# flavie-yuan-liu/DL_attack_on_ImageNet

Measured on AMD Instinct MI355X. Metric: adversarial images/sec (ADiL learning step, classifier included), higher is better.
Workload: dtype bf16; 1 GPU; ADiL learn_dictionary_a step vs resnet50, 512 images/GPU, 50 atoms, 224x224, bf16 image streams + fp32 D/V master, loss=logits, clean pseudo-labels computed once per image and cached (1 fwd + 1 bwd per step; result-neutral, profiles/r03_label_stability.md); global_batch=512, atoms=50, inner_iters=131, parallelism=dp1: images+codes sharded, D replicated, 1 all-reduce(grad_d)/step

## Files before the change

### dl_attack_on_imagenet_amd/_lib.py

```python
import ctypes
import os
from ctypes import c_float, c_int, c_size_t, c_void_p

_PKG = os.path.dirname(os.path.abspath(__file__))
LIBPATH = os.environ.get("ADIL_HIP_LIBRARY") or os.path.join(_PKG, "lib", "libadil_hip.so")

SIGNATURES = {
    "adil_abi_version": (c_int, []),
    "adil_max_atoms": (c_int, []),
    "adil_grad_workspace_bytes": (c_size_t, [c_int, c_int, c_int]),
    "adil_grad_code_rows": (c_int, [c_int]),
    "adil_grad_slab_offset": (c_size_t, [c_int, c_int, c_int]),
    "adil_pack_codes": (c_int, [c_void_p, c_void_p, c_int, c_int, c_void_p, c_void_p, c_void_p, c_int, c_void_p, c_int, c_int,
                                c_void_p]),
    "adil_gather_images": (c_int, [c_void_p, c_int, c_void_p, c_void_p, c_int, c_int, c_int, c_void_p]),
    "adil_spd_inverse": (c_int, [c_void_p, c_int, c_void_p, c_void_p]),
    "adil_synth": (c_int, [c_void_p, c_void_p, c_void_p, c_void_p, c_int, c_int, c_int, c_int, c_float, c_int, c_void_p]),
    "adil_images_to_u8": (c_int, [c_void_p, c_int, c_void_p, c_size_t, c_void_p, c_void_p]),
    "adil_synth_store": (c_int, [c_void_p, c_void_p, c_void_p, c_void_p, c_void_p, c_int, c_int, c_int, c_int, c_float, c_int,
                                 c_void_p]),
    "adil_synth_fp8": (c_int, [c_void_p, c_void_p, c_void_p, c_void_p, c_int, c_int, c_int, c_int, c_float, c_float, c_int,
                               c_void_p]),
    "adil_dict_to_fp8": (c_int, [c_void_p, c_size_t, c_void_p, c_void_p]),
    "adil_adamw_clamp_fp8": (c_int, [c_void_p, c_void_p, c_int, c_void_p, c_void_p, c_size_t, c_float, c_float, c_float,
                                     c_float, c_float, c_float, c_float, c_float, c_void_p, c_void_p, c_void_p, c_void_p]),
    "adil_synth_fp8_packed": (c_int, [c_void_p, c_void_p, c_void_p, c_void_p, c_int, c_int, c_int, c_int, c_float, c_float,
                                      c_int, c_void_p]),
    "adil_grad": (c_int, [c_void_p, c_void_p, c_void_p, c_void_p, c_void_p, c_void_p, c_int, c_int, c_int, c_int, c_int,
                          c_void_p, c_size_t, c_void_p, c_void_p]),
    "adil_adamw_clamp": (c_int, [c_void_p, c_void_p, c_int, c_void_p, c_void_p, c_size_t, c_float, c_float, c_float,
                                 c_float, c_float, c_float, c_float, c_float, c_void_p, c_void_p, c_void_p]),
    "adil_zstep": (c_int, [c_void_p, c_void_p, c_void_p, c_void_p, c_void_p, c_int, c_int, c_int, c_float, c_float,
                           c_float, c_float, c_float, c_float, c_float, c_float, c_void_p, c_void_p, c_float, c_void_p,
                           c_void_p, c_void_p]),
    "adil_zstep_codes_slab_bytes": (c_size_t, [c_int, c_int, c_int]),
    "adil_zstep_codes": (c_int, [c_void_p, c_void_p, c_void_p, c_void_p, c_void_p, c_int, c_int, c_int, c_float, c_float,
                                 c_float, c_float, c_float, c_float, c_float, c_float, c_void_p, c_void_p, c_float, c_void_p,
                                 c_void_p, c_void_p, c_size_t, c_void_p, c_void_p]),
    "adil_adamw_l1ball": (c_int, [c_void_p, c_void_p, c_void_p, c_int, c_void_p, c_void_p, c_int, c_int, c_float, c_float,
                                  c_float, c_float, c_float, c_float, c_float, c_void_p, c_void_p, c_float, c_void_p, c_void_p,
                                  c_void_p, c_int, c_int, c_void_p]),
    "adil_atom_l1ball_project": (c_int, [c_void_p, c_int, c_int, c_int, c_float, c_void_p]),
    "adil_l1ball_project": (c_int, [c_void_p, c_int, c_int, c_float, c_void_p]),
    "adil_l2ball_project": (c_int, [c_void_p, c_int, c_int, c_float, c_void_p]),
    "adil_ista_step": (c_int, [c_void_p, c_void_p, c_size_t, c_float, c_float, c_void_p]),
    "adil_atom_workspace_bytes": (c_size_t, [c_int, c_int]),
    "adil_atom_norms": (c_int, [c_void_p, c_int, c_int, c_void_p, c_void_p, c_size_t, c_void_p]),
    "adil_atom_scale": (c_int, [c_void_p, c_int, c_int, c_void_p, c_int, c_void_p]),
    "adil_gram_workspace_bytes": (c_size_t, [c_int, c_int]),
    "adil_gram": (c_int, [c_void_p, c_int, c_int, c_void_p, c_void_p, c_size_t, c_void_p]),
    "adil_dict_rightmul": (c_int, [c_void_p, c_void_p, c_int, c_int, c_void_p, c_void_p]),
    "adil_image_metrics": (c_int, [c_void_p, c_void_p, c_int, c_int, c_int, c_void_p, c_void_p, c_void_p]),
    "adil_affine_act_fwd": (c_int, [c_void_p, c_void_p, c_void_p, c_void_p, c_void_p, c_size_t, c_int, c_int, c_int, c_int,
                                    c_void_p]),
    "adil_affine_act_bwd": (c_int, [c_void_p, c_void_p, c_void_p, c_void_p, c_void_p, c_size_t, c_int, c_int, c_int, c_int,
                                    c_void_p]),
    "adil_stem_conv_fwd": (c_int, [c_void_p, c_int, c_void_p, c_float, c_float, c_float, c_float, c_float, c_float,
                                   c_void_p, c_void_p, c_void_p, c_int, c_int, c_int, c_void_p]),
    "adil_maxpool_fwd": (c_int, [c_void_p, c_void_p, c_void_p, c_int, c_int, c_int, c_int, c_void_p]),
    "adil_stem_pool_bwd": (c_int, [c_void_p, c_void_p, c_void_p, c_void_p, c_void_p, c_int, c_int, c_int, c_int, c_void_p]),
    "adil_pw_conv_fwd": (c_int, [c_void_p, c_void_p, c_void_p, c_void_p, c_void_p, c_void_p, c_int, c_int, c_int, c_int,
                                 c_void_p, c_void_p, c_int, c_int, c_void_p]),
    "adil_pw_conv_bwd": (c_int, [c_void_p, c_void_p, c_void_p, c_void_p, c_void_p, c_void_p, c_void_p, c_int, c_int, c_int,
                                 c_int, c_void_p, c_void_p, c_void_p, c_void_p, c_int, c_int, c_void_p]),
    "adil_pw_conv_bwd_tile": (c_int, [c_void_p, c_void_p, c_void_p, c_void_p, c_void_p, c_void_p, c_void_p, c_int, c_int, c_int,
                                      c_int, c_void_p, c_void_p, c_void_p, c_void_p, c_int, c_int, c_void_p, c_int]),
    "adil_pw_route_policy": (c_int, [c_int]),
    "adil_pw_join_fwd": (c_int, [c_void_p, c_void_p, c_void_p, c_void_p, c_void_p, c_void_p, c_void_p, c_void_p, c_void_p,
                                 c_void_p, c_void_p, c_void_p, c_int, c_int, c_int, c_void_p]),
    "adil_pw_join_bwd": (c_int, [c_void_p, c_void_p, c_void_p, c_void_p, c_void_p, c_void_p, c_void_p, c_void_p, c_void_p,
                                 c_void_p, c_void_p, c_void_p, c_void_p, c_int, c_int, c_int, c_void_p]),
    "adil_conv3x3": (c_int, [c_void_p, c_void_p, c_void_p, c_int, c_int, c_int, c_int, c_int, c_void_p]),
    "adil_conv3x3_loop": (c_int, [c_int]),
    "adil_conv3x3_s2_fwd": (c_int, [c_void_p, c_void_p, c_void_p, c_int, c_int, c_int, c_int, c_int, c_void_p]),
    "adil_conv3x3_s2_bwd": (c_int, [c_void_p, c_void_p, c_void_p, c_int, c_int, c_int, c_int, c_int, c_void_p]),
    "adil_dw3x3_fwd": (c_int, [c_void_p, c_void_p, c_void_p, c_void_p, c_int, c_int, c_int, c_int, c_int, c_int, c_void_p]),
    "adil_dw3x3_bwd": (c_int, [c_void_p, c_void_p, c_void_p, c_void_p, c_int, c_int, c_int, c_int, c_int, c_int, c_void_p]),
    "adil_pw8_fwd": (c_int, [c_void_p, c_void_p, c_void_p, c_void_p, c_void_p, c_void_p, c_int, c_int, c_int, c_int, c_void_p]),
    "adil_pw8_bwd": (c_int, [c_void_p, c_void_p, c_void_p, c_void_p, c_void_p, c_int, c_int, c_int, c_int, c_void_p]),
    "adil_stem_conv_bwd": (c_int, [c_void_p, c_void_p, c_float, c_float, c_float, c_void_p, c_int, c_int, c_int, c_int,
                                   c_void_p]),
    "adil_stem_bwd_variant": (c_int, [c_int]),
    "adil_first3x3_fwd": (c_int, [c_void_p, c_int, c_void_p, c_float, c_float, c_float, c_float, c_float, c_float,
                                  c_void_p, c_void_p, c_void_p, c_int, c_int, c_int, c_int, c_void_p]),
    "adil_first3x3_bwd": (c_int, [c_void_p, c_void_p, c_void_p, c_void_p, c_float, c_float, c_float, c_void_p, c_int, c_int,
                                  c_int, c_int, c_int, c_void_p]),
    "adil_pool_head_fwd": (c_int, [c_void_p, c_void_p, c_void_p, c_void_p, c_void_p, c_int, c_int, c_int, c_int, c_void_p]),
    "adil_pool_head_bwd": (c_int, [c_void_p, c_void_p, c_void_p, c_void_p, c_int, c_int, c_int, c_int, c_void_p]),
    "adil_bn_pool_head_fwd": (c_int, [c_void_p] * 7 + [c_int, c_int, c_int, c_int, c_void_p]),
    "adil_bn_pool_head_bwd": (c_int, [c_void_p] * 7 + [c_int, c_int, c_int, c_int, c_void_p]),
    "adil_dense1x1_fwd": (c_int, [c_void_p, c_void_p, c_void_p, c_void_p, c_void_p, c_void_p, c_void_p, c_int, c_int, c_int,
                                  c_int, c_void_p]),
    "adil_dense1x1_bwd": (c_int, [c_void_p, c_void_p, c_void_p, c_void_p, c_void_p, c_void_p, c_void_p, c_void_p, c_int, c_int,
                                  c_int, c_int, c_void_p]),
    "adil_dense3x3_fwd": (c_int, [c_void_p, c_void_p, c_void_p, c_int, c_int, c_int, c_int, c_int, c_void_p]),
    "adil_dense3x3_bwd": (c_int, [c_void_p, c_void_p, c_void_p, c_int, c_int, c_int, c_int, c_int, c_void_p]),
    "adil_dense1x1_fwd_ld": (c_int, [c_void_p, c_int, c_void_p, c_void_p, c_void_p, c_void_p, c_void_p, c_void_p, c_int, c_int,
                                     c_int, c_int, c_int, c_void_p]),
    "adil_dense1x1_bwd_ld": (c_int, [c_void_p, c_int, c_void_p, c_int, c_void_p, c_void_p, c_void_p, c_int, c_void_p, c_void_p,
                                     c_void_p, c_int, c_int, c_int, c_int, c_int, c_int, c_void_p]),
    "adil_dense3x3_fwd_ld": (c_int, [c_void_p, c_int, c_void_p, c_void_p, c_int, c_int, c_int, c_int, c_int, c_int, c_void_p]),
    "adil_dense3x3_bwd_ld": (c_int, [c_void_p, c_int, c_void_p, c_void_p, c_int, c_int, c_int, c_int, c_int, c_int, c_void_p]),
    "adil_dense_transition_fwd": (c_int, [c_void_p, c_void_p, c_void_p, c_void_p, c_void_p, c_int, c_int, c_int, c_int, c_int,
                                          c_void_p]),
    "adil_dense_transition_bwd": (c_int, [c_void_p, c_int, c_void_p, c_void_p, c_void_p, c_void_p, c_void_p, c_int, c_int,
                                          c_int, c_int, c_int, c_void_p]),
}

ABI_VERSION = 8
_lib = None


class AdilLibraryError(RuntimeError):
    pass


def load(path: str = None) -> ctypes.CDLL:
    global _lib
    if _lib is not None and path is None:
        return _lib
    p = path or LIBPATH
    import torch
    if not os.path.exists(p):
        raise AdilLibraryError(
            f"HIP kernel library not found at {p}. Build it with `python -m dl_attack_on_imagenet_amd.build` "
            "(needs hipcc). There is no CPU fallback for the ADiL hot path.")
# ... 22 lines not shown
```

### dl_attack_on_imagenet_amd/csrc/adil_convs.hip

```cpp
#include <hip/hip_runtime.h>
#include <stdint.h>

#include "adil_common.h"
#include "adil_hip.h"
#include "adil_mfma.h"

namespace {

#define PW_BM 128
#define PW_BK 64
#define PW_LS (PW_BK + 8)
#define PW_PK 512

template <int BN, bool PRO, bool RES>
__global__ __launch_bounds__(256) __attribute__((amdgpu_waves_per_eu(PRO && BN == 128 ? 2 : (RES ? 3 : 4)))) void pw_conv_fwd_kernel(
    const bf16_t* __restrict__ x, const bf16_t* __restrict__ wgt, const float* __restrict__ scale,
    const float* __restrict__ shift, const bf16_t* __restrict__ res, bf16_t* __restrict__ y, int M, int K, int N,
    int relu, int MT, int NT, const float* __restrict__ pscale, const float* __restrict__ pshift, int sub_w, int sub_hw) {
    constexpr int CT = BN / 32;
    constexpr int XCH = PW_BM * PW_BK / 8 / 256;
    constexpr int WCH = BN * PW_BK / 8 / 256;
    constexpr int OS = BN + 8;
    extern __shared__ __attribute__((aligned(16))) unsigned char smem_raw[];
    bf16_t* sx = reinterpret_cast<bf16_t*>(smem_raw);
// ... 695 lines not shown
}

template <int WD, bool BWD>
int launch_pw_join(const JoinArgs& a, hipStream_t st) {
    const size_t lds = ((size_t)(PW_BM + 64) * (WD + 8) + (size_t)(WD + PW_BM) * PW_LS) * sizeof(bf16_t);
    if (lds > 48 * 1024) {
        const hipError_t e = hipFuncSetAttribute((const void*)pw_join_kernel<WD, BWD>,
                                                 hipFuncAttributeMaxDynamicSharedMemorySize, (int)lds);
        if (e != hipSuccess) return (int)e;
    }
    hipLaunchKernelGGL((pw_join_kernel<WD, BWD>), dim3((unsigned)((a.M + PW_BM - 1) / PW_BM)), dim3(256), lds, st, a);
    ADIL_CHECK_LAUNCH();
    return 0;
}

template <bool BWD>
int launch_pw_join_w(const JoinArgs& a, int W, hipStream_t st) {
    if (W == 64) return launch_pw_join<64, BWD>(a, st);
    return launch_pw_join<128, BWD>(a, st);
}

}

extern "C" int adil_pw_join_fwd(const void* h2raw, const float* pscale2, const float* pshift2, const void* w3,
                                const float* scale3, const float* shift3, const void* res, void* out, const void* w1,
                                const float* scale1, const float* shift1, void* h1, int M, int W, int C, void* stream) {
    ADIL_ENTER();
    if (!h2raw || !pscale2 || !pshift2 || !w3 || !scale3 || !shift3 || !res || !out || !w1 || !scale1 || !shift1 || !h1 ||
        M <= 0 || (W != 64 && W != 128) || C != 4 * W)
        return ADIL_EINVAL;
    const JoinArgs a = {(const bf16_t*)h2raw, nullptr, pscale2, pshift2, (const bf16_t*)w3, scale3, shift3,
                        (const bf16_t*)res, nullptr, (bf16_t*)out, (const bf16_t*)w1, scale1, shift1, nullptr, (bf16_t*)h1,
                        M, C};
    return launch_pw_join_w<false>(a, W, (hipStream_t)stream);
}

extern "C" int adil_pw_join_bwd(const void* g_h1, const void* h1, const float* scale1, const void* wt1, const void* g_out,
                                const void* out, const float* scale3, void* gres, const void* wt3, const void* h2raw,
                                const float* pscale2, const float* pshift2, void* gx, int M, int W, int C, void* stream) {
    ADIL_ENTER();
    if (!g_h1 || !h1 || !scale1 || !wt1 || !g_out || !out || !scale3 || !gres || !wt3 || !h2raw || !pscale2 || !pshift2 ||
        !gx || M <= 0 || (W != 64 && W != 128) || C != 4 * W)
        return ADIL_EINVAL;
    const JoinArgs a = {(const bf16_t*)g_h1, (const bf16_t*)h1, scale1, nullptr, (const bf16_t*)wt1, scale3, nullptr,
                        (const bf16_t*)g_out, (const bf16_t*)out, (bf16_t*)gres, (const bf16_t*)wt3, pscale2, pshift2,
                        (const bf16_t*)h2raw, (bf16_t*)gx, M, C};
    return launch_pw_join_w<true>(a, W, (hipStream_t)stream);
}

namespace {

#define C3_LS 72

template <int BN, int WPX, int LOOP>
__global__ __launch_bounds__(256) __attribute__((amdgpu_waves_per_eu(2))) void conv3x3_kernel(
    const bf16_t* __restrict__ x, const bf16_t* __restrict__ wp, bf16_t* __restrict__ y, int M, int H, int W, int C, int N,
    int MT, int NT) {
    constexpr int C3_BM = WPX * 64;
    constexpr int CTW = BN / 32 / (4 / WPX);
    constexpr int XCHK = (C3_BM + 128) * 8 / 256;
    constexpr int WCH = BN * 8 / 256;
    constexpr int OS = BN + 8;
    extern __shared__ __attribute__((aligned(16))) unsigned char smem_raw[];
    const int NP = C3_BM + 2 * W + 2;
    bf16_t* sx = reinterpret_cast<bf16_t*>(smem_raw);
    const int sx_elems = (NP * C3_LS > C3_BM * OS ? NP * C3_LS : C3_BM * OS);
    bf16_t* sw = sx + ((sx_elems + 7) & ~7);
    const int tid = threadIdx.x, lane = tid & 63, w = tid >> 6, c = lane & 31, h = lane >> 5;
    const int wpx = w % WPX, wch = w / WPX;
    int mt, nt;
    if ((MT & 7) == 0) {
        const int xcd = blockIdx.x & 7, j = blockIdx.x >> 3;
        nt = j % NT;
        mt = (j / NT) * 8 + xcd;
    } else {
        nt = blockIdx.x % NT;
        mt = blockIdx.x / NT;
    }
    const int m0 = mt * C3_BM, n0 = nt * BN;
    const int nci = C >> 6;

    int pl[2];
    unsigned vmask[2];
#pragma unroll
    for (int p = 0; p < 2; ++p) {
        pl[p] = (wpx * 2 + p) * 32 + c;
        const int m = m0 + pl[p];
        const int ww = m % W, hh = (m / W) % H;
        unsigned vm = 0;
#pragma unroll
        for (int t = 0; t < 9; ++t) {
            const int kh = t / 3, kw = t - 3 * kh;
            const bool ok = (m < M) && (hh + kh - 1 >= 0) && (hh + kh - 1 < H) && (ww + kw - 1 >= 0) && (ww + kw - 1 < W);
            vm |= ok ? (1u << t) : 0u;
        }
        vmask[p] = vm;
    }

    u32x4 xr[XCHK], wr[3][WCH];
    [[maybe_unused]] auto load_x = [&](int cc) {
#pragma unroll
        for (int i = 0; i < XCHK; ++i) {
            const int q = tid + 256 * i, px = q >> 3, ch = q & 7;
            int gm = m0 - W - 1 + (px < NP ? px : NP - 1);
            gm = gm < 0 ? 0 : (gm >= M ? M - 1 : gm);
            xr[i] = *reinterpret_cast<const u32x4*>(x + (size_t)gm * C + cc * 64 + ch * 8);
        }
    };
    auto store_x = [&]() {
#pragma unroll
        for (int i = 0; i < XCHK; ++i) {
            const int q = tid + 256 * i, px = q >> 3, ch = q & 7;
            if (px < NP) *reinterpret_cast<u32x4*>(sx + px * C3_LS + ch * 8) = xr[i];
        }
    };
    const int nit = nci * 9;
    [[maybe_unused]] auto load_w = [&](int it, u32x4 (&r)[WCH]) {
        const int itc = it < nit ? it : nit - 1;
        const int cc = itc / 9, tap = itc - 9 * cc;
#pragma unroll
        for (int i = 0; i < WCH; ++i) {
            const int q = tid + 256 * i, row = q >> 3, ch = q & 7;
            r[i] = *reinterpret_cast<const u32x4*>(wp + ((size_t)(n0 + row) * 9 + tap) * C + cc * 64 + ch * 8);
        }
    };
    auto store_w = [&](int buf, const u32x4 (&r)[WCH]) {
#pragma unroll
        for (int i = 0; i < WCH; ++i) {
            const int q = tid + 256 * i, row = q >> 3, ch = q & 7;
            *reinterpret_cast<u32x4*>(sw + (buf * BN + row) * C3_LS + ch * 8) = r[i];
        }
    };

    f32x16 acc[2][CTW];
#pragma unroll
    for (int p = 0; p < 2; ++p)
#pragma unroll
        for (int ct = 0; ct < CTW; ++ct)
#pragma unroll
            for (int r = 0; r < 16; ++r) acc[p][ct][r] = 0.0f;

    if constexpr (LOOP == 1) {
        auto tap_body = [&](int it, u32x4 (&rfree)[WCH], const u32x4 (&rnext)[WCH]) {
            const int buf = it & 1;
            const int cc = it / 9, tap = it - 9 * cc;
            const int kh = tap / 3, kw = tap - 3 * kh;
            load_w(it + 3, rfree);
            if (tap == 4 && cc + 1 < nci) load_x(cc + 1);
            const bf16_t* bw = sw + (buf * BN + (wch * CTW) * 32 + c) * C3_LS + 8 * h;
            const int shift = kh * W + kw;
            const bool ok0 = (vmask[0] >> tap) & 1u, ok1 = (vmask[1] >> tap) & 1u;
#pragma unroll
            for (int ks = 0; ks < 4; ++ks) {
                bf16x8 b0 = lds8(sx + (pl[0] + shift) * C3_LS + 16 * ks + 8 * h);
                bf16x8 b1 = lds8(sx + (pl[1] + shift) * C3_LS + 16 * ks + 8 * h);
                u32x4 z0 = __builtin_bit_cast(u32x4, b0), z1 = __builtin_bit_cast(u32x4, b1);
#pragma unroll
                for (int j = 0; j < 4; ++j) { z0[j] = ok0 ? z0[j] : 0u; z1[j] = ok1 ? z1[j] : 0u; }
                b0 = __builtin_bit_cast(bf16x8, z0);
                b1 = __builtin_bit_cast(bf16x8, z1);
#pragma unroll
                for (int ct = 0; ct < CTW; ++ct) {
                    const bf16x8 a = lds8(bw + ct * 32 * C3_LS + 16 * ks);
                    mma16(acc[0][ct], a, b0);
                    mma16(acc[1][ct], a, b1);
                }
            }
            if (it + 1 < nit) store_w(buf ^ 1, rnext);
            if (tap == 8 && cc + 1 < nci) {
                lds_barrier();
                store_x();
            }
            lds_barrier();
        };

        load_x(0);
        load_w(0, wr[0]);
        load_w(1, wr[1]);
        load_w(2, wr[2]);
        store_x();
        store_w(0, wr[0]);
        __syncthreads();
        for (int it = 0; it < nit; it += 3) {
            tap_body(it, wr[0], wr[1]);
            tap_body(it + 1, wr[1], wr[2]);
            tap_body(it + 2, wr[2], wr[0]);
        }
    } else {
        const unsigned wq = (((unsigned)(n0 + (tid >> 3)) * 9u) * (unsigned)C + (unsigned)(tid & 7) * 8u) * 2u;
        const size_t wrow = (size_t)32 * 9 * C;
        auto load_w0 = [&](unsigned ws, u32x4 (&r)[WCH]) {
#pragma unroll
            for (int i = 0; i < WCH; ++i)
                r[i] = *reinterpret_cast<const u32x4*>(reinterpret_cast<const char*>(wp + ws + i * wrow) + wq);
        };
        const int gmb = m0 - W - 1 > 0 ? m0 - W - 1 : 0;
        const bf16_t* xb = x + (size_t)gmb * C;
        unsigned xq[XCHK];
#pragma unroll
        for (int i = 0; i < XCHK; ++i) {
            const int px = (tid >> 3) + 32 * i;
            int gm = m0 - W - 1 + (px < NP ? px : NP - 1);
            gm = gm < 0 ? 0 : (gm >= M ? M - 1 : gm);
            xq[i] = ((unsigned)(gm - gmb) * (unsigned)C + (unsigned)(tid & 7) * 8u) * 2u;
        }
        auto load_x0 = [&](int cc) {
#pragma unroll
            for (int i = 0; i < XCHK; ++i)
                xr[i] = *reinterpret_cast<const u32x4*>(reinterpret_cast<const char*>(xb + cc * 64) + xq[i]);
        };
        bf16_t* sz = sw + 2 * BN * C3_LS;
        const bf16_t* xl0 = sx + pl[0] * C3_LS + 8 * h;
        const bf16_t* xl1 = sx + pl[1] * C3_LS + 8 * h;
        const bf16_t* zl = sz + 8 * h;
        const bf16_t* bwl = sw + ((wch * CTW) * 32 + c) * C3_LS + 8 * h;
        auto xrow = [&](const bf16_t* xl, unsigned vm, int tap) -> const bf16_t* {
            const int kh = tap / 3, kw = tap - 3 * kh;
            const bf16_t* a = xl + (kh * W + kw) * C3_LS;
            if (tap == 4) return a;
            return (vm & (1u << tap)) ? a : zl;
        };
        struct Frag {
            bf16x8 b0, b1, a[CTW];
        };
        auto read_frag = [&](Frag& f, const bf16_t* p0, const bf16_t* p1, const bf16_t* bw, int ks) {
            f.b0 = lds8(p0 + 16 * ks);
            f.b1 = lds8(p1 + 16 * ks);
#pragma unroll
            for (int ct = 0; ct < CTW; ++ct) f.a[ct] = lds8(bw + ct * 32 * C3_LS + 16 * ks);
        };
        auto mma_frag = [&](const Frag& f) {
#pragma unroll
            for (int ct = 0; ct < CTW; ++ct) {
                mma16(acc[0][ct], f.a[ct], f.b0);
                mma16(acc[1][ct], f.a[ct], f.b1);
            }
        };

        load_x0(0);
        load_w0(0u, wr[0]);
        load_w0((unsigned)C, wr[1]);
        load_w0(2u * (unsigned)C, wr[2]);
        store_x();
        store_w(0, wr[0]);
        if (tid < C3_LS / 8) reinterpret_cast<u32x4*>(sz)[tid] = u32x4{0u, 0u, 0u, 0u};
        __syncthreads();
        Frag fa, fb;
        const bf16_t* p0 = xrow(xl0, vmask[0], 0);
        const bf16_t* p1 = xrow(xl1, vmask[1], 0);
        read_frag(fa, p0, p1, bwl, 0);
        for (int cc = 0; cc < nci; ++cc) {
            const bool more = cc + 1 < nci;
            const unsigned wsc = (unsigned)cc * 64u, wsn = (unsigned)(more ? cc + 1 : cc) * 64u;
#pragma unroll
            for (int tap = 0; tap < 9; ++tap) {
                const int buf = (cc + tap) & 1;
                const bf16_t* bw = bwl + buf * BN * C3_LS;
                const bool last = !more && tap == 8;
                read_frag(fb, p0, p1, bw, 1);
                if (!last) store_w(buf ^ 1, wr[(tap + 1) % 3]);
                load_w0(tap + 3 < 9 ? wsc + (unsigned)((tap + 3) * C) : wsn + (unsigned)((tap - 6) * C), wr[tap % 3]);
                if (tap == 4 && more) load_x0(cc + 1);
                __builtin_amdgcn_sched_barrier(0);
                mma_frag(fa);
                __builtin_amdgcn_sched_barrier(0);
                read_frag(fa, p0, p1, bw, 2);
                __builtin_amdgcn_sched_barrier(0);
                mma_frag(fb);
                __builtin_amdgcn_sched_barrier(0);
                read_frag(fb, p0, p1, bw, 3);
                __builtin_amdgcn_sched_barrier(0);
                mma_frag(fa);
                __builtin_amdgcn_sched_barrier(0);
                lds_barrier();
                if (tap == 8 && more) {
                    store_x();
                    lds_barrier();
                }
                if (!last) {
                    p0 = xrow(xl0, vmask[0], (tap + 1) % 9);
                    p1 = xrow(xl1, vmask[1], (tap + 1) % 9);
                    read_frag(fa, p0, p1, bwl + (buf ^ 1) * BN * C3_LS, 0);
                }
                __builtin_amdgcn_sched_barrier(0);
                mma_frag(fb);
                __builtin_amdgcn_sched_barrier(0);
            }
        }
    }
#pragma unroll
    for (int p = 0; p < 2; ++p) {
#pragma unroll
        for (int ct = 0; ct < CTW; ++ct) {
#pragma unroll
            for (int q = 0; q < 4; ++q) {
                u32x2 t;
                t[0] = pack2_bf16(acc[p][ct][4 * q], acc[p][ct][4 * q + 1]);
                t[1] = pack2_bf16(acc[p][ct][4 * q + 2], acc[p][ct][4 * q + 3]);
                *reinterpret_cast<u32x2*>(sx + pl[p] * OS + (wch * CTW + ct) * 32 + 8 * q + 4 * h) = t;
            }
        }
    }
    __syncthreads();
    constexpr int CPP = BN / 8;
#pragma unroll
    for (int i = 0; i < C3_BM * CPP / 256; ++i) {
        const int id = tid + 256 * i, px = id / CPP, ch = id - px * CPP;
        const int mm = m0 + px;
        if (mm < M) *reinterpret_cast<u32x4*>(y + (size_t)mm * N + n0 + ch * 8) = *reinterpret_cast<const u32x4*>(sx + px * OS + ch * 8);
    }
}

template <int BN, int WPX, int LOOP>
int launch_conv3x3(const void* x, const void* wp, void* y, int M, int H, int W, int C, int N, hipStream_t st) {
    constexpr int C3_BM = WPX * 64;
    const int MT = (M + C3_BM - 1) / C3_BM, NT = N / BN;
    const int NP = C3_BM + 2 * W + 2;
    size_t sx_elems = (size_t)NP * C3_LS;
    if (sx_elems < (size_t)C3_BM * (BN + 8)) sx_elems = (size_t)C3_BM * (BN + 8);
    sx_elems = (sx_elems + 7) & ~(size_t)7;
    const size_t lds = (sx_elems + (size_t)2 * BN * C3_LS + (LOOP == 0 ? C3_LS : 0)) * sizeof(bf16_t);
    if (lds > 160 * 1024) return ADIL_EINVAL;
    if (lds > 48 * 1024) {
        const hipError_t e = hipFuncSetAttribute((const void*)conv3x3_kernel<BN, WPX, LOOP>,
                                                 hipFuncAttributeMaxDynamicSharedMemorySize, (int)lds);
        if (e != hipSuccess) return (int)e;
    }
    hipLaunchKernelGGL((conv3x3_kernel<BN, WPX, LOOP>), dim3((unsigned)(MT * NT)), dim3(256), lds, st, (const bf16_t*)x,
                       (const bf16_t*)wp, (bf16_t*)y, M, H, W, C, N, MT, NT);
    ADIL_CHECK_LAUNCH();
    return 0;
}

static int g_conv3x3_loop = 0;

}

extern "C" int adil_conv3x3_loop(int variant) {
    const int prev = g_conv3x3_loop;
    if (variant == 0 || variant == 1) g_conv3x3_loop = variant;
    return prev;
}

extern "C" int adil_conv3x3(const void* x, const void* wp, void* y, int B, int H, int W, int C, int N, void* stream) {
    ADIL_ENTER();
    if (!x || !wp || !y || B <= 0 || H <= 0 || W <= 0 || C <= 0 || N <= 0 || (C % 64) || (N % 64) || W > 63) return ADIL_EINVAL;
    const long long M = (long long)B * H * W;
    if (M > 0x7fffffffLL) return ADIL_EINVAL;
    if (9LL * C * N > 0x7fffffffLL) return ADIL_EINVAL;
    const hipStream_t st = (hipStream_t)stream;
    if (g_conv3x3_loop == 1) {
        if (N % 128 == 0) return launch_conv3x3<128, 2, 1>(x, wp, y, (int)M, H, W, C, N, st);
        return launch_conv3x3<64, 4, 1>(x, wp, y, (int)M, H, W, C, N, st);
    }
    if (N % 128 == 0) return launch_conv3x3<128, 2, 0>(x, wp, y, (int)M, H, W, C, N, st);
    return launch_conv3x3<64, 4, 0>(x, wp, y, (int)M, H, W, C, N, st);
}

namespace {

#define S2_BM 128

template <int BN, bool BWD, int LOOP>
__global__ __launch_bounds__(256) __attribute__((amdgpu_waves_per_eu(2))) void conv3x3_s2_kernel(
    const bf16_t* __restrict__ src, const bf16_t* __restrict__ wp, bf16_t* __restrict__ dst, int M, int OH, int OW, int K,
    int NO, int MT, int NT) {
    constexpr int CTW = BN / 64;
    constexpr int XCH = S2_BM * 8 / 256;
    constexpr int WCH = BN * 8 / 256;
    constexpr int OS = BN + 8;
    constexpr int PAIR = (S2_BM + BN) * C3_LS;
    constexpr int NCLS = BWD ? 4 : 1;
    constexpr bool PIPE = LOOP == 0 && BN == 64;
    static_assert(S2_BM * OS <= PAIR, "the output transpose goes through one idle buffer");
    extern __shared__ __attribute__((aligned(16))) unsigned char smem_raw[];
    bf16_t* sb = reinterpret_cast<bf16_t*>(smem_raw);
    const int tid = threadIdx.x, lane = tid & 63, w = tid >> 6, c = lane & 31, h = lane >> 5;
    const int wpx = w & 1, wch = w >> 1;
    int mt, nt;
    if ((MT & 7) == 0) {
        const int xcd = blockIdx.x & 7, j = blockIdx.x >> 3;
        nt = j % NT;
        mt = (j / NT) * 8 + xcd;
    } else {
        nt = blockIdx.x % NT;
        mt = blockIdx.x / NT;
    }
    const int m0 = mt * S2_BM, n0 = nt * BN;
    const int nci = K >> 6;
    const int nit = nci * 9;
    auto cls_ph = [](int cls) { return BWD ? (cls < 2 ? 1 : 0) : 0; };
    auto cls_pw = [](int cls) { return BWD ? ((cls & 1) ? 0 : 1) : 0; };

    int ctr[XCH];
    unsigned flg[XCH];
#pragma unroll
    for (int i = 0; i < XCH; ++i) {
        const int r = m0 + (tid >> 3) + 32 * i;
        const int rc = r < M ? r : M - 1;
        const int j = rc % OW, ii = (rc / OW) % OH;
        ctr[i] = BWD ? rc : 4 * rc - 2 * j;
        const bool okh = BWD ? (ii + 1 < OH) : (ii > 0), okw = BWD ? (j + 1 < OW) : (j > 0);
        flg[i] = (r < M ? 1u : 0u) | (okh ? 2u : 0u) | (okw ? 4u : 0u);
    }
    struct Tile {
        u32x4 x[XCH], w[WCH];
        unsigned ok;
    };
    int lcls = 0, lcc = 0, la = 0, lb = 0;
// ... 260 lines not shown
```

### include/adil_hip.h

```cpp
#ifndef ADIL_HIP_H
#define ADIL_HIP_H

#include <stddef.h>
#include <stdint.h>

#ifdef __cplusplus
extern "C" {
#endif

#define ADIL_F32 0
#define ADIL_BF16 1
#define ADIL_U8 2

#define ADIL_EINVAL (-1)
#define ADIL_EWORKSPACE (-2)

int adil_abi_version(void);

int adil_max_atoms(void);

size_t adil_grad_workspace_bytes(int B, int P, int K);

int adil_grad_code_rows(int K);

// ... 52 lines not shown
int adil_l2ball_project(float* x, int N, int K, float radius, void* stream);

int adil_ista_step(float* v, const float* g, size_t n, float step, float lam, void* stream);

size_t adil_atom_workspace_bytes(int P, int K);
int adil_atom_norms(const float* d, int P, int K, float* norms, void* ws, size_t ws_bytes, void* stream);

int adil_atom_scale(float* d, int P, int K, const float* norms, int sphere, void* stream);

size_t adil_gram_workspace_bytes(int P, int K);
int adil_gram(const float* d, int P, int K, float* gram, void* ws, size_t ws_bytes, void* stream);

int adil_spd_inverse(const float* a, int K, float* out, void* stream);

int adil_dict_rightmul(const float* d, const float* mat, int P, int K, float* out, void* stream);

int adil_image_metrics(const void* adv, const void* x, int B, int P, int dtype, float* sq_err, float* sq_norm,
                       void* stream);

int adil_affine_act_fwd(const void* x, const void* res, const float* scale, const float* shift, void* y, size_t n, int C,
                        int inner, int relu, int dtype, void* stream);
int adil_affine_act_bwd(const void* g, const void* y, const float* scale, void* gx, void* gres, size_t n, int C,
                        int inner, int relu, int dtype, void* stream);

int adil_stem_conv_fwd(const void* x, int x_dtype, const void* w_fwd, float mean0, float mean1, float mean2, float inv_std0,
                       float inv_std1, float inv_std2, const float* scale, const float* shift, void* y, int B, int H, int W,
                       void* stream);
int adil_maxpool_fwd(const void* y, void* p, uint8_t* idx, int B, int OH, int OW, int C, void* stream);
int adil_stem_pool_bwd(const void* g, const uint8_t* idx, const void* p, const float* scale, void* gy, int B, int OH, int OW,
                       int C, void* stream);
int adil_stem_conv_bwd(const void* gy, const void* w_bwd, float inv_std0, float inv_std1, float inv_std2, void* gx,
                       int gx_dtype, int B, int H, int W, void* stream);
int adil_stem_bwd_variant(int variant);

int adil_pw_conv_fwd(const void* x, const void* w, const float* scale, const float* shift, const void* res, void* y, int M,
                     int K, int N, int relu, const float* pscale, const float* pshift, int sub_w, int sub_hw, void* stream);
int adil_pw_conv_bwd(const void* g, const void* g2, const void* y, const float* scale, const void* wt, void* gx, void* gres,
                     int M, int K, int N, int relu, const void* xin, const float* pscale, const float* pshift, const void* g3,
                     int sub_w, int sub_hw, void* stream);
int adil_pw_conv_bwd_tile(const void* g, const void* g2, const void* y, const float* scale, const void* wt, void* gx,
                          void* gres, int M, int K, int N, int relu, const void* xin, const float* pscale,
                          const float* pshift, const void* g3, int sub_w, int sub_hw, void* stream, int bo);
int adil_pw_route_policy(int policy);
int adil_conv3x3_loop(int variant);

int adil_pw_join_fwd(const void* h2raw, const float* pscale2, const float* pshift2, const void* w3, const float* scale3,
                     const float* shift3, const void* res, void* out, const void* w1, const float* scale1,
                     const float* shift1, void* h1, int M, int W, int C, void* stream);
int adil_pw_join_bwd(const void* g_h1, const void* h1, const float* scale1, const void* wt1, const void* g_out,
                     const void* out, const float* scale3, void* gres, const void* wt3, const void* h2raw,
                     const float* pscale2, const float* pshift2, void* gx, int M, int W, int C, void* stream);

int adil_conv3x3(const void* x, const void* wp, void* y, int B, int H, int W, int C, int N, void* stream);

#define ADIL_CONV3X3_S2_MAX_W 63
int adil_conv3x3_s2_fwd(const void* x, const void* wp, void* y, int B, int H, int W, int C, int N, void* stream);
int adil_conv3x3_s2_bwd(const void* g, const void* wp_bwd, void* gx, int B, int H, int W, int C, int N, void* stream);

int adil_dw3x3_fwd(const void* x, const float* w, const float* bias, void* y, int B, int H, int W, int C, int stride,
                   int relu6, void* stream);
int adil_dw3x3_bwd(const void* g, const void* y, const float* w, void* gx, int B, int H, int W, int C, int stride,
                   int relu6, void* stream);

int adil_pw8_fwd(const void* x, const void* w, const float* scale, const float* shift, const void* res, void* y, int M,
                 int K, int N, int act, void* stream);
int adil_pw8_bwd(const void* g, const void* y, const float* scale, const void* wt, void* gx, int M, int K, int N, int act,
                 void* stream);

int adil_first3x3_fwd(const void* x, int x_dtype, const void* w_fwd, float mean0, float mean1, float mean2, float inv_std0,
                      float inv_std1, float inv_std2, const float* scale, const float* shift, void* y, int B, int H, int W,
                      int relu6, void* stream);
int adil_first3x3_bwd(const void* g, const void* y, const float* scale, const void* w_bwd, float inv_std0, float inv_std1,
                      float inv_std2, void* gx, int gx_dtype, int B, int H, int W, int relu6, void* stream);

int adil_pool_head_fwd(const void* x, const float* wt, const float* bias, float* pooled, float* logits, int B, int HW,
                       int C, int N, void* stream);
int adil_pool_head_bwd(const float* g, const float* w, float* gpooled, void* gx, int B, int HW, int C, int N, void* stream);

int adil_bn_pool_head_fwd(const void* x, const float* pscale, const float* pshift, const float* wt, const float* bias,
                          float* pooled, float* logits, int B, int HW, int C, int N, void* stream);
int adil_bn_pool_head_bwd(const float* g, const float* w, const void* x, const float* pscale, const float* pshift,
                          float* gpooled, void* gx, int B, int HW, int C, int N, void* stream);

int adil_dense1x1_fwd(const void* x, const float* pscale, const float* pshift, const void* w, const float* scale,
                      const float* shift, void* y, int M, int K, int N, int act, void* stream);
int adil_dense1x1_bwd(const void* g, const void* y, const float* scale, const void* wt, const void* xin, const float* pscale,
                      const float* pshift, void* gx, int M, int K, int N, int act, void* stream);
int adil_dense1x1_fwd_ld(const void* x, int ldx, const float* pscale, const float* pshift, const void* w,
                         const float* scale, const float* shift, void* y, int ldy,
                         int M, int K, int N, int act, void* stream);
int adil_dense1x1_bwd_ld(const void* g, int ldg, const void* y, int ldy, const float* scale, const void* wt,
                         const void* xin, int ldxin, const float* pscale, const float* pshift,
                         void* gx, int ldgx, int accumulate, int M, int K, int N, int act, void* stream);

#define ADIL_DENSE3X3_MAX_W 63
int adil_dense3x3_fwd(const void* x, const void* wp, void* y, int B, int H, int W, int C, int N, void* stream);
int adil_dense3x3_bwd(const void* g, const void* wp_bwd, void* gx, int B, int H, int W, int C, int N, void* stream);
int adil_dense3x3_fwd_ld(const void* x, int ldx, const void* wp, void* y, int ldy,
                         int B, int H, int W, int C, int N, void* stream);
int adil_dense3x3_bwd_ld(const void* g, int ldg, const void* wp_bwd, void* gx, int ldgx,
                         int B, int H, int W, int C, int N, void* stream);

int adil_dense_transition_fwd(const void* x, const float* pscale, const float* pshift, const void* w, void* y,
                              int B, int H, int W, int K, int N, void* stream);
int adil_dense_transition_bwd(const void* g, int ldg, const void* wt, const void* xin, const float* pscale,
                              const float* pshift, void* gx, int B, int H, int W, int K, int N, void* stream);
// ... 6 lines not shown
```

Before: 25990 images/sec.

## Add 8-wave and persistent tile-walking variants of the 3x3 conv kernel

New measurement: 26200 images/sec, median of 6. No clear change (+0.8%).

```diff
diff --git a/dl_attack_on_imagenet_amd/_lib.py b/dl_attack_on_imagenet_amd/_lib.py
--- a/dl_attack_on_imagenet_amd/_lib.py
+++ b/dl_attack_on_imagenet_amd/_lib.py
@@ -72,6 +72,8 @@
                                  c_void_p, c_void_p, c_void_p, c_void_p, c_int, c_int, c_int, c_void_p]),
     "adil_conv3x3": (c_int, [c_void_p, c_void_p, c_void_p, c_int, c_int, c_int, c_int, c_int, c_void_p]),
     "adil_conv3x3_loop": (c_int, [c_int]),
+    "adil_conv3x3_form": (c_int, [c_void_p, c_void_p, c_void_p, c_int, c_int, c_int, c_int, c_int, c_void_p, c_int, c_int]),
+    "adil_conv3x3_policy": (c_int, [c_int]),
     "adil_conv3x3_s2_fwd": (c_int, [c_void_p, c_void_p, c_void_p, c_int, c_int, c_int, c_int, c_int, c_void_p]),
     "adil_conv3x3_s2_bwd": (c_int, [c_void_p, c_void_p, c_void_p, c_int, c_int, c_int, c_int, c_int, c_void_p]),
     "adil_dw3x3_fwd": (c_int, [c_void_p, c_void_p, c_void_p, c_void_p, c_int, c_int, c_int, c_int, c_int, c_int, c_void_p]),
diff --git a/dl_attack_on_imagenet_amd/csrc/adil_convs.hip b/dl_attack_on_imagenet_amd/csrc/adil_convs.hip
--- a/dl_attack_on_imagenet_amd/csrc/adil_convs.hip
+++ b/dl_attack_on_imagenet_amd/csrc/adil_convs.hip
@@ -771,14 +771,16 @@
 
 #define C3_LS 72
 
-template <int BN, int WPX, int LOOP>
-__global__ __launch_bounds__(256) __attribute__((amdgpu_waves_per_eu(2))) void conv3x3_kernel(
+template <int BN, int WPX, int LOOP, int NW = 4, int WALK = 0>
+__global__ __launch_bounds__(NW * 64) __attribute__((amdgpu_waves_per_eu(2))) void conv3x3_kernel(
     const bf16_t* __restrict__ x, const bf16_t* __restrict__ wp, bf16_t* __restrict__ y, int M, int H, int W, int C, int N,
     int MT, int NT) {
+    static_assert(LOOP == 0 || (NW == 4 && WALK == 0), "the step loop keeps the 4-wave tiles, one tile per workgroup");
+    constexpr int NTH = NW * 64;
     constexpr int C3_BM = WPX * 64;
-    constexpr int CTW = BN / 32 / (4 / WPX);
-    constexpr int XCHK = (C3_BM + 128) * 8 / 256;
-    constexpr int WCH = BN * 8 / 256;
+    constexpr int CTW = BN / 32 / (NW / WPX);
+    constexpr int XCHK = (C3_BM + 128) * 8 / NTH;
+    constexpr int WCH = BN * 8 / NTH;
     constexpr int OS = BN + 8;
     extern __shared__ __attribute__((aligned(16))) unsigned char smem_raw[];
     const int NP = C3_BM + 2 * W + 2;
@@ -787,8 +789,9 @@
     bf16_t* sw = sx + ((sx_elems + 7) & ~7);
     const int tid = threadIdx.x, lane = tid & 63, w = tid >> 6, c = lane & 31, h = lane >> 5;
     const int wpx = w % WPX, wch = w / WPX;
+    const int MS = WALK ? (int)gridDim.x / NT : MT;
     int mt, nt;
-    if ((MT & 7) == 0) {
+    if ((MS & 7) == 0) {
         const int xcd = blockIdx.x & 7, j = blockIdx.x >> 3;
         nt = j % NT;
         mt = (j / NT) * 8 + xcd;
@@ -796,31 +799,43 @@
         nt = blockIdx.x % NT;
         mt = blockIdx.x / NT;
     }
-    const int m0 = mt * C3_BM, n0 = nt * BN;
+    [[maybe_unused]] int tl = mt, tl1 = mt + 1;
+    if constexpr (WALK) {
+        tl = (int)((long long)mt * MT / MS);
+        tl1 = (int)((long long)(mt + 1) * MT / MS);
+        if (tl >= tl1) return;
+        mt = tl;
+    }
+    int m0 = mt * C3_BM;
+    const int n0 = nt * BN;
     const int nci = C >> 6;
 
     int pl[2];
     unsigned vmask[2];
 #pragma unroll
-    for (int p = 0; p < 2; ++p) {
-        pl[p] = (wpx * 2 + p) * 32 + c;
-        const int m = m0 + pl[p];
-        const int ww = m % W, hh = (m / W) % H;
-        unsigned vm = 0;
-#pragma unroll
-        for (int t = 0; t < 9; ++t) {
-            const int kh = t / 3, kw = t - 3 * kh;
-            const bool ok = (m < M) && (hh + kh - 1 >= 0) && (hh + kh - 1 < H) && (ww + kw - 1 >= 0) && (ww + kw - 1 < W);
-            vm |= ok ? (1u << t) : 0u;
-        }
-        vmask[p] = vm;
-    }
+    for (int p = 0; p < 2; ++p) pl[p] = (wpx * 2 + p) * 32 + c;
+    auto set_vmask = [&]() {
+#pragma unroll
+        for (int p = 0; p < 2; ++p) {
+            const int m = m0 + pl[p];
+            const int ww = m % W, hh = (m / W) % H;
+            unsigned vm = 0;
+#pragma unroll
+            for (int t = 0; t < 9; ++t) {
+                const int kh = t / 3, kw = t - 3 * kh;
+                const bool ok = (m < M) && (hh + kh - 1 >= 0) && (hh + kh - 1 < H) && (ww + kw - 1 >= 0) && (ww + kw - 1 < W);
+                vm |= ok ? (1u << t) : 0u;
+            }
+            vmask[p] = vm;
+        }
+    };
+    set_vmask();
 
     u32x4 xr[XCHK], wr[3][WCH];
     [[maybe_unused]] auto load_x = [&](int cc) {
 #pragma unroll
         for (int i = 0; i < XCHK; ++i) {
-            const int q = tid + 256 * i, px = q >> 3, ch = q & 7;
+            const int q = tid + NTH * i, px = q >> 3, ch = q & 7;
             int gm = m0 - W - 1 + (px < NP ? px : NP - 1);
             gm = gm < 0 ? 0 : (gm >= M ? M - 1 : gm);
             xr[i] = *reinterpret_cast<const u32x4*>(x + (size_t)gm * C + cc * 64 + ch * 8);
@@ -829,7 +844,7 @@
     auto store_x = [&]() {
 #pragma unroll
         for (int i = 0; i < XCHK; ++i) {
-            const int q = tid + 256 * i, px = q >> 3, ch = q & 7;
+            const int q = tid + NTH * i, px = q >> 3, ch = q & 7;
             if (px < NP) *reinterpret_cast<u32x4*>(sx + px * C3_LS + ch * 8) = xr[i];
         }
     };
@@ -839,25 +854,56 @@
         const int cc = itc / 9, tap = itc - 9 * cc;
 #pragma unroll
         for (int i = 0; i < WCH; ++i) {
-            const int q = tid + 256 * i, row = q >> 3, ch = q & 7;
+            const int q = tid + NTH * i, row = q >> 3, ch = q & 7;
             r[i] = *reinterpret_cast<const u32x4*>(wp + ((size_t)(n0 + row) * 9 + tap) * C + cc * 64 + ch * 8);
         }
     };
     auto store_w = [&](int buf, const u32x4 (&r)[WCH]) {
 #pragma unroll
         for (int i = 0; i < WCH; ++i) {
-            const int q = tid + 256 * i, row = q >> 3, ch = q & 7;
+            const int q = tid + NTH * i, row = q >> 3, ch = q & 7;
             *reinterpret_cast<u32x4*>(sw + (buf * BN + row) * C3_LS + ch * 8) = r[i];
         }
     };
 
     f32x16 acc[2][CTW];
-#pragma unroll
-    for (int p = 0; p < 2; ++p)
-#pragma unroll
-        for (int ct = 0; ct < CTW; ++ct)
-#pragma unroll
-            for (int r = 0; r < 16; ++r) acc[p][ct][r] = 0.0f;
+    auto zero_acc = [&]() {
+#pragma unroll
+        for (int p = 0; p < 2; ++p)
+#pragma unroll
+            for (int ct = 0; ct < CTW; ++ct)
+#pragma unroll
+                for (int r = 0; r < 16; ++r) acc[p][ct][r] = 0.0f;
+    };
+    if constexpr (!WALK) zero_acc();
+    auto write_tile = [&]() {
+#pragma unroll
+        for (int p = 0; p < 2; ++p) {
+#pragma unroll
+            for (int ct = 0; ct < CTW; ++ct) {
+#pragma unroll
+                for (int q = 0; q < 4; ++q) {
+                    u32x2 t;
+                    t[0] = pack2_bf16(acc[p][ct][4 * q], acc[p][ct][4 * q + 1]);
+                    t[1] = pack2_bf16(acc[p][ct][4 * q + 2], acc[p][ct][4 * q + 3]);
+                    *reinterpret_cast<u32x2*>(sx + pl[p] * OS + (wch * CTW + ct) * 32 + 8 * q + 4 * h) = t;
+                }
+            }
+        }
+        __syncthreads();
+        constexpr int CPP = BN / 8, RPS = NTH / CPP;
+        int ts = tid;
+        if constexpr (WALK) asm volatile("" : "+v"(ts));
+        const int px0 = ts / CPP, ch = ts - px0 * CPP;
+        const unsigned yq = ((unsigned)px0 * (unsigned)N + (unsigned)ch * 8u) * 2u;
+        char* yb = reinterpret_cast<char*>(y + (size_t)m0 * N + n0);
+        const bf16_t* so = sx + px0 * OS + ch * 8;
+        const int left = M - m0 - px0;
+#pragma unroll
+        for (int i = 0; i < C3_BM / RPS; ++i)
+            if (i * RPS < left)
+                *reinterpret_cast<u32x4*>(yb + (size_t)i * RPS * N * 2 + yq) = *reinterpret_cast<const u32x4*>(so + i * RPS * OS);
+    };
 
     if constexpr (LOOP == 1) {
         auto tap_body = [&](int it, u32x4 (&rfree)[WCH], const u32x4 (&rnext)[WCH]) {
@@ -907,26 +953,36 @@
         }
     } else {
         const unsigned wq = (((unsigned)(n0 + (tid >> 3)) * 9u) * (unsigned)C + (unsigned)(tid & 7) * 8u) * 2u;
-        const size_t wrow = (size_t)32 * 9 * C;
+        const size_t wrow = (size_t)(NTH / 8) * 9 * C;
         auto load_w0 = [&](unsigned ws, u32x4 (&r)[WCH]) {
 #pragma unroll
             for (int i = 0; i < WCH; ++i)
                 r[i] = *reinterpret_cast<const u32x4*>(reinterpret_cast<const char*>(wp + ws + i * wrow) + wq);
         };
-        const int gmb = m0 - W - 1 > 0 ? m0 - W - 1 : 0;
-        const bf16_t* xb = x + (size_t)gmb * C;
-        unsigned xq[XCHK];
-#pragma unroll
-        for (int i = 0; i < XCHK; ++i) {
-            const int px = (tid >> 3) + 32 * i;
-            int gm = m0 - W - 1 + (px < NP ? px : NP - 1);
+        int xm = m0;
+        auto xoff = [&](int i, int ts) -> unsigned {
+            const int gmb = xm - W - 1 > 0 ? xm - W - 1 : 0;
+            const int px = (ts >> 3) + (NTH / 8) * i;
+            int gm = xm - W - 1 + (px < NP ? px : NP - 1);
             gm = gm < 0 ? 0 : (gm >= M ? M - 1 : gm);
-            xq[i] = ((unsigned)(gm - gmb) * (unsigned)C + (unsigned)(tid & 7) * 8u) * 2u;
+            return ((unsigned)(gm - gmb) * (unsigned)C + (unsigned)(ts & 7) * 8u) * 2u;
+        };
+        [[maybe_unused]] unsigned xq[WALK ? 1 : XCHK];
+        if constexpr (!WALK) {
+#pragma unroll
+            for (int i = 0; i < XCHK; ++i) xq[i] = xoff(i, tid);
         }
         auto load_x0 = [&](int cc) {
-#pragma unroll
-            for (int i = 0; i < XCHK; ++i)
-                xr[i] = *reinterpret_cast<const u32x4*>(reinterpret_cast<const char*>(xb + cc * 64) + xq[i]);
+            const int gmb = xm - W - 1 > 0 ? xm - W - 1 : 0;
+            const char* xb = reinterpret_cast<const char*>(x + (size_t)gmb * C + cc * 64);
+            [[maybe_unused]] int ts = tid;
+            if constexpr (WALK) asm volatile("" : "+v"(ts));
+#pragma unroll
+            for (int i = 0; i < XCHK; ++i) {
+                unsigned q;
+                if constexpr (WALK) q = xoff(i, ts); else q = xq[i];
+                xr[i] = *reinterpret_cast<const u32x4*>(xb + q);
+            }
         };
         bf16_t* sz = sw + 2 * BN * C3_LS;
         const bf16_t* xl0 = sx + pl[0] * C3_LS + 8 * h;
@@ -968,18 +1024,30 @@
         const bf16_t* p0 = xrow(xl0, vmask[0], 0);
         const bf16_t* p1 = xrow(xl1, vmask[1], 0);
         read_frag(fa, p0, p1, bwl, 0);
+        [[maybe_unused]] int par = 0;
+        for (;;) {
+        if constexpr (WALK) zero_acc();
+        [[maybe_unused]] bool nextt = false;
         for (int cc = 0; cc < nci; ++cc) {
             const bool more = cc + 1 < nci;
-            const unsigned wsc = (unsigned)cc * 64u, wsn = (unsigned)(more ? cc + 1 : cc) * 64u;
+            if constexpr (WALK) nextt = !more && tl + 1 < tl1;
+            const unsigned wsc = (unsigned)cc * 64u;
+            const unsigned wsn = more ? wsc + 64u : (nextt ? 0u : wsc);
 #pragma unroll
             for (int tap = 0; tap < 9; ++tap) {
-                const int buf = (cc + tap) & 1;
+                const int buf = (WALK ? par + cc + tap : cc + tap) & 1;
                 const bf16_t* bw = bwl + buf * BN * C3_LS;
-                const bool last = !more && tap == 8;
+                const bool last = !more && !nextt && tap == 8;
                 read_frag(fb, p0, p1, bw, 1);
                 if (!last) store_w(buf ^ 1, wr[(tap + 1) % 3]);
                 load_w0(tap + 3 < 9 ? wsc + (unsigned)((tap + 3) * C) : wsn + (unsigned)((tap - 6) * C), wr[tap % 3]);
                 if (tap == 4 && more) load_x0(cc + 1);
+                if constexpr (WALK) {
+                    if (tap == 4 && nextt) {
+                        xm = m0 + C3_BM;
+                        load_x0(0);
+                    }
+                }
                 __builtin_amdgcn_sched_barrier(0);
                 mma_frag(fa);
                 __builtin_amdgcn_sched_barrier(0);
@@ -996,7 +1064,7 @@
                     store_x();
                     lds_barrier();
                 }
-                if (!last) {
+                if (!last && !(WALK && tap == 8 && nextt)) {
                     p0 = xrow(xl0, vmask[0], (tap + 1) % 9);
                     p1 = xrow(xl1, vmask[1], (tap + 1) % 9);
                     read_frag(fa, p0, p1, bwl + (buf ^ 1) * BN * C3_LS, 0);
@@ -1006,31 +1074,31 @@
                 __builtin_amdgcn_sched_barrier(0);
             }
         }
-    }
-#pragma unroll
-    for (int p = 0; p < 2; ++p) {
-#pragma unroll
-        for (int ct = 0; ct < CTW; ++ct) {
-#pragma unroll
-            for (int q = 0; q < 4; ++q) {
-                u32x2 t;
-                t[0] = pack2_bf16(acc[p][ct][4 * q], acc[p][ct][4 * q + 1]);
-                t[1] = pack2_bf16(acc[p][ct][4 * q + 2], acc[p][ct][4 * q + 3]);
-                *reinterpret_cast<u32x2*>(sx + pl[p] * OS + (wch * CTW + ct) * 32 + 8 * q + 4 * h) = t;
-            }
-        }
-    }
-    __syncthreads();
-    constexpr int CPP = BN / 8;
-#pragma unroll
-    for (int i = 0; i < C3_BM * CPP / 256; ++i) {
-        const int id = tid + 256 * i, px = id / CPP, ch = id - px * CPP;
-        const int mm = m0 + px;
-        if (mm < M) *reinterpret_cast<u32x4*>(y + (size_t)mm * N + n0 + ch * 8) = *reinterpret_cast<const u32x4*>(sx + px * OS + ch * 8);
-    }
-}
-
-template <int BN, int WPX, int LOOP>
+        if constexpr (!WALK) {
+            break;
+        } else {
+            write_tile();
+            if (!nextt) return;
+            __syncthreads();
+            store_x();
+            ++tl;
+            m0 += C3_BM;
+            par = (par + nci) & 1;
+            asm volatile("" : "+v"(pl[0]), "+v"(pl[1]));
+            xl0 = sx + pl[0] * C3_LS + 8 * h;
+            xl1 = sx + pl[1] * C3_LS + 8 * h;
+            set_vmask();
+            lds_barrier();
+            p0 = xrow(xl0, vmask[0], 0);
+            p1 = xrow(xl1, vmask[1], 0);
+            read_frag(fa, p0, p1, bwl + par * BN * C3_LS, 0);
+        }
+        }
+    }
+    write_tile();
+}
+
+template <int BN, int WPX, int LOOP, int NW = 4, int WALK = 0>
 int launch_conv3x3(const void* x, const void* wp, void* y, int M, int H, int W, int C, int N, hipStream_t st) {
     constexpr int C3_BM = WPX * 64;
     const int MT = (M + C3_BM - 1) / C3_BM, NT = N / BN;
@@ -1041,17 +1109,82 @@
     const size_t lds = (sx_elems + (size_t)2 * BN * C3_LS + (LOOP == 0 ? C3_LS : 0)) * sizeof(bf16_t);
     if (lds > 160 * 1024) return ADIL_EINVAL;
     if (lds > 48 * 1024) {
-        const hipError_t e = hipFuncSetAttribute((const void*)conv3x3_kernel<BN, WPX, LOOP>,
+        const hipError_t e = hipFuncSetAttribute((const void*)conv3x3_kernel<BN, WPX, LOOP, NW, WALK>,
                                                  hipFuncAttributeMaxDynamicSharedMemorySize, (int)lds);
         if (e != hipSuccess) return (int)e;
     }
-    hipLaunchKernelGGL((conv3x3_kernel<BN, WPX, LOOP>), dim3((unsigned)(MT * NT)), dim3(256), lds, st, (const bf16_t*)x,
-                       (const bf16_t*)wp, (bf16_t*)y, M, H, W, C, N, MT, NT);
+    long long grid = (long long)MT * NT;
+    if (WALK) {
+        int per = 8 / NW;
+        if ((size_t)per * lds > 160 * 1024) per = (int)(160 * 1024 / lds);
+        int slots = adil_num_cu() * per / NT;
+        if (slots >= 8) slots &= ~7;
+        if (slots < 1) slots = 1;
+        if (slots > MT) slots = (((MT + 7) & ~7) <= slots) ? ((MT + 7) & ~7) : MT;
+        grid = (long long)slots * NT;
+    }
+    hipLaunchKernelGGL((conv3x3_kernel<BN, WPX, LOOP, NW, WALK>), dim3((unsigned)grid), dim3(NW * 64), lds, st,
+                       (const bf16_t*)x, (const bf16_t*)wp, (bf16_t*)y, M, H, W, C, N, MT, NT);
     ADIL_CHECK_LAUNCH();
     return 0;
 }
 
 static int g_conv3x3_loop = 0;
+
+static int g_conv3x3_policy = 0;
+
+struct Conv3x3Row { int C, N, m_lo, m_hi, nw, walk; };
+static const Conv3x3Row kConv3x3Forms[] = {
+    {128, 128, 401408, INT32_MAX, 8, 1},
+    {128, 128, 100352, 200703, 8, 1},
+    {128, 128, 50176, 100351, 8, 0},
+    {256, 256, 50176, 100351, 8, 1},
+    {512, 512, 25088, INT32_MAX, 8, 1},
+    {512, 512, 12544, 25087, 8, 0},
+};
+
+static void conv3x3_pick(int M, int C, int N, int* nw, int* walk) {
+    *nw = 4;
+    *walk = 0;
+    if (g_conv3x3_policy == 1) return;
+    if (g_conv3x3_policy == 2) {
+        *nw = 8;
+        *walk = 1;
+        return;
+    }
+    for (const Conv3x3Row& r : kConv3x3Forms)
+        if (r.C == C && r.N == N && M >= r.m_lo && M <= r.m_hi) {
+            *nw = r.nw;
+            *walk = r.walk;
+            return;
+        }
+}
+
+static int conv3x3_check(const void* x, const void* wp, void* y, int B, int H, int W, int C, int N, long long* M) {
+    if (!x || !wp || !y || B <= 0 || H <= 0 || W <= 0 || C <= 0 || N <= 0 || (C % 64) || (N % 64) || W > 63) return ADIL_EINVAL;
+    *M = (long long)B * H * W;
+    if (*M > 0x7fffffffLL) return ADIL_EINVAL;
+    if (9LL * C * N > 0x7fffffffLL) return ADIL_EINVAL;
+    return 0;
+}
+
+static int conv3x3_run(int nw, int walk, const void* x, const void* wp, void* y, int M, int H, int W, int C, int N, hipStream_t st) {
+    if (g_conv3x3_loop == 1) {
+        if (nw != 4 || walk) return ADIL_EINVAL;
+        if (N % 128 == 0) return launch_conv3x3<128, 2, 1>(x, wp, y, M, H, W, C, N, st);
+        return launch_conv3x3<64, 4, 1>(x, wp, y, M, H, W, C, N, st);
+    }
+    if (N % 128 == 0) {
+        if (nw == 8) return walk ? launch_conv3x3<128, 4, 0, 8, 1>(x, wp, y, M, H, W, C, N, st)
+                                 : launch_conv3x3<128, 4, 0, 8, 0>(x, wp, y, M, H, W, C, N, st);
+        return walk ? launch_conv3x3<128, 2, 0, 4, 1>(x, wp, y, M, H, W, C, N, st)
+                    : launch_conv3x3<128, 2, 0, 4, 0>(x, wp, y, M, H, W, C, N, st);
+    }
+    if (nw == 8) return walk ? launch_conv3x3<64, 8, 0, 8, 1>(x, wp, y, M, H, W, C, N, st)
+                             : launch_conv3x3<64, 8, 0, 8, 0>(x, wp, y, M, H, W, C, N, st);
+    return walk ? launch_conv3x3<64, 4, 0, 4, 1>(x, wp, y, M, H, W, C, N, st)
+                : launch_conv3x3<64, 4, 0, 4, 0>(x, wp, y, M, H, W, C, N, st);
+}
 
 }
 
@@ -1063,17 +1196,26 @@
 
 extern "C" int adil_conv3x3(const void* x, const void* wp, void* y, int B, int H, int W, int C, int N, void* stream) {
     ADIL_ENTER();
-    if (!x || !wp || !y || B <= 0 || H <= 0 || W <= 0 || C <= 0 || N <= 0 || (C % 64) || (N % 64) || W > 63) return ADIL_EINVAL;
-    const long long M = (long long)B * H * W;
-    if (M > 0x7fffffffLL) return ADIL_EINVAL;
-    if (9LL * C * N > 0x7fffffffLL) return ADIL_EINVAL;
-    const hipStream_t st = (hipStream_t)stream;
-    if (g_conv3x3_loop == 1) {
-        if (N % 128 == 0) return launch_conv3x3<128, 2, 1>(x, wp, y, (int)M, H, W, C, N, st);
-        return launch_conv3x3<64, 4, 1>(x, wp, y, (int)M, H, W, C, N, st);
-    }
-    if (N % 128 == 0) return launch_conv3x3<128, 2, 0>(x, wp, y, (int)M, H, W, C, N, st);
-    return launch_conv3x3<64, 4, 0>(x, wp, y, (int)M, H, W, C, N, st);
+    long long M = 0;
+    if (conv3x3_check(x, wp, y, B, H, W, C, N, &M)) return ADIL_EINVAL;
+    int nw = 4, walk = 0;
+    if (g_conv3x3_loop == 0) conv3x3_pick((int)M, C, N, &nw, &walk);
+    return conv3x3_run(nw, walk, x, wp, y, (int)M, H, W, C, N, (hipStream_t)stream);
+}
+
+extern "C" int adil_conv3x3_form(const void* x, const void* wp, void* y, int B, int H, int W, int C, int N, void* stream,
+                                 int nw, int walk) {
+    ADIL_ENTER();
+    long long M = 0;
+    if (conv3x3_check(x, wp, y, B, H, W, C, N, &M)) return ADIL_EINVAL;
+    if ((nw != 4 && nw != 8) || (walk != 0 && walk != 1)) return ADIL_EINVAL;
+    return conv3x3_run(nw, walk, x, wp, y, (int)M, H, W, C, N, (hipStream_t)stream);
+}
+
+extern "C" int adil_conv3x3_policy(int policy) {
+    const int prev = g_conv3x3_policy;
+    if (policy >= 0 && policy <= 2) g_conv3x3_policy = policy;
+    return prev;
 }
 
 namespace {
diff --git a/include/adil_hip.h b/include/adil_hip.h
--- a/include/adil_hip.h
+++ b/include/adil_hip.h
@@ -128,6 +128,9 @@
                      const float* pscale2, const float* pshift2, void* gx, int M, int W, int C, void* stream);
 
 int adil_conv3x3(const void* x, const void* wp, void* y, int B, int H, int W, int C, int N, void* stream);
+int adil_conv3x3_form(const void* x, const void* wp, void* y, int B, int H, int W, int C, int N, void* stream, int nw,
+                      int walk);
+int adil_conv3x3_policy(int policy);
 
 #define ADIL_CONV3X3_S2_MAX_W 63
 int adil_conv3x3_s2_fwd(const void* x, const void* wp, void* y, int B, int H, int W, int C, int N, void* stream);
```
